# jeongminpark417/COALA-GNN

Measured on AMD Instinct MI355X. Metric: feature-gather GB/s (payload = rows x dim x 4 B delivered per second), IGB-medium GraphSAGE minibatch fetch, higher is better.
Workload: dtype f32

## Files before the change

coala-gnn_amd/csrc/coala_cache.hip:

```cpp
#include <hip/hip_runtime.h>
#include <hip/hip_ext.h>

#include <algorithm>
#include <cmath>
#include <cstdarg>
#include <cstdio>
#include <cstdlib>
#include <cstring>
#include <new>
#include <type_traits>
#include <utility>
#include <vector>

#include "../../include/coala_hip.h"
#include "coala_internal.h"

namespace {

constexpr uint64_t kEmptyKey = 0xFFFFFFFFFFFFFFFFull;
constexpr uint32_t kLinkMiss = 0x80000000u;
constexpr uint32_t kLinkBad = 0x7FFFFFFFu;
constexpr int kStatBlocks = 2048;
constexpr int kFillSlots = 8;

struct CacheDev {
    void* keys;
    uint64_t* set_cnt;
    uint32_t* color_meta;
    int32_t* color_counters;
    const int32_t* node_color;
    float* lines;
    const float* cold;
    uint64_t num_sets;
    uint64_t num_rows;
    uint32_t cache_dim;
    uint32_t dim;
    uint32_t n_gpus;
    int32_t gshift;
    int32_t sshift;
    uint32_t distributed;
    uint32_t cold_partitioned;
    uint32_t tag32;
    uint64_t* set_head;
    uint32_t* miss_link;
    unsigned long long* stats;
    uint32_t* miss_list;
    uint32_t list_sub;
};

constexpr int kListShards = 64;
constexpr int kListStride = 64;
constexpr int kStatWriteBad = 2 * kStatBlocks + kFillSlots + 1;
constexpr int kStatProbeBad = kStatWriteBad + 1;
constexpr int kStatHostWords = kStatProbeBad + 1;
constexpr int kStatList = (kStatHostWords + 31) & ~31;
constexpr int kStatWords = kStatList + 2 * kListShards * kListStride / 2;
__device__ __forceinline__ uint32_t* list_counter(const CacheDev& c, uint32_t parity, uint32_t shard) {
    return reinterpret_cast<uint32_t*>(c.stats + kStatList) + (parity * kListShards + shard) * kListStride;
}

__device__ __forceinline__ uint64_t set_of(const CacheDev& c, uint64_t id) {
    uint64_t k = id;
    if (c.distributed) {
        if (c.gshift >= 0) k = id >> c.gshift;
        else if ((id >> 32) == 0) k = (uint32_t)id / c.n_gpus;
        else k = id / c.n_gpus;
    }
    if (c.sshift >= 0) return k & (c.num_sets - 1);
    if ((k >> 32) == 0 && (c.num_sets >> 32) == 0) return (uint32_t)k % (uint32_t)c.num_sets;
    return k % c.num_sets;
}

__device__ __forceinline__ uint64_t cold_row_of(const CacheDev& c, uint64_t id) {
    if (!c.cold_partitioned) return id;
    if (c.gshift >= 0) return id >> c.gshift;
    return id / c.n_gpus;
}

constexpr int kMaxRanges = 64;
struct RangeSet {
    uint32_t n;
    uint32_t total;
    uint32_t begin[kMaxRanges];
    uint32_t vstart[kMaxRanges + 1];
};
__device__ __forceinline__ uint32_t pos_of(const RangeSet& rs, uint32_t v) {
    if (rs.n == 1) return v < rs.total ? rs.begin[0] + v : 0xFFFFFFFFu;
    uint32_t pos = 0xFFFFFFFFu;
    for (uint32_t k = 0; k < rs.n; ++k) {
        const uint32_t a = rs.vstart[k], b = rs.vstart[k + 1];
        if (v >= a && v < b) pos = rs.begin[k] + (v - a);
    }
    return pos;
}
struct Redirect {
    int64_t begin, end;
    float* out;
    const int64_t* row_map;
};

template <int CTRL> __device__ __forceinline__ uint32_t dpp_u32(uint32_t v) {
    return (uint32_t)__builtin_amdgcn_mov_dpp((int)v, CTRL, 0xF, 0xF, true);
}
__device__ __forceinline__ uint32_t umin_u32(uint32_t a, uint32_t b) { return a < b ? a : b; }
__device__ __forceinline__ uint64_t readlane64(uint64_t v, int src_lane) {
    uint32_t lo = __builtin_amdgcn_readlane((int)(uint32_t)v, src_lane);
    uint32_t hi = __builtin_amdgcn_readlane((int)(uint32_t)(v >> 32), src_lane);
    return ((uint64_t)hi << 32) | lo;
}

__device__ __forceinline__ uint64_t shfl64(uint64_t v, int src) {
    const uint32_t lo = __shfl((int)(uint32_t)v, src), hi = __shfl((int)(uint32_t)(v >> 32), src);
    return ((uint64_t)hi << 32) | lo;
}

typedef float vfloat4 __attribute__((ext_vector_type(4)));
typedef unsigned long long vu64x2 __attribute__((ext_vector_type(2)));
typedef unsigned int vu32x4 __attribute__((ext_vector_type(4)));

template <typename TAG> struct TagGeo;
template <> struct TagGeo<uint64_t> {
    using vec = vu64x2;
    static constexpr int KPL = 2;
    static constexpr int LPS = 16;
    static constexpr int SPL = 4;
    static constexpr uint64_t EMPTY = 0xFFFFFFFFFFFFFFFFull;
};
template <> struct TagGeo<uint32_t> {
    using vec = vu32x4;
    static constexpr int KPL = 4;
    static constexpr int LPS = 8;
    static constexpr int SPL = 8;
    static constexpr uint32_t EMPTY = 0xFFFFFFFFu;
};
template <int VEC> struct VecT;
template <> struct VecT<4> { using type = vfloat4; };
template <> struct VecT<1> { using type = float; };

template <int CD, int VEC, int NP = 4>
struct Geo {
    static constexpr int UNITS = CD / VEC;
    static constexpr int LPR = UNITS >= 64 ? 64 : UNITS;
    static constexpr int RPP = 64 / LPR;
    static constexpr int VPL = UNITS / LPR;
    static constexpr int PASSES = (VPL >= 16) ? 1 : NP;
    static constexpr int R = RPP * PASSES;
};

constexpr int kK1MinWaves = 4;
constexpr int kK1Passes = 4;
constexpr int64_t kK1SingleMaxChunks = 1 << 20;
constexpr int kK1Waves = 2;
#ifdef COALA_DEV_KNOBS
constexpr int kK1MaxWaves = 4;
#else
constexpr int kK1MaxWaves = kK1Waves;
#endif

template <typename V> __device__ __forceinline__ V nt_load(const V* p) { return __builtin_nontemporal_load(p); }
template <typename V> __device__ __forceinline__ void nt_store(V v, V* p) { __builtin_nontemporal_store(v, p); }

template <int CD, int VEC, typename TAG, int NP, bool FULL, bool REDIR, bool SINGLE>
__global__ __launch_bounds__(64 * kK1MaxWaves, kK1MinWaves) void probe_gather_kernel(const int64_t* __restrict__ idx, float* __restrict__ out,
                                                                    int64_t n, uint32_t gen, uint32_t n_blocks, CacheDev c, Redirect rd) {
    using G = Geo<CD, VEC, NP>;
    using V = typename VecT<VEC>::type;
    using TG = TagGeo<TAG>;
    using TV = typename TG::vec;
    constexpr int R = G::R;
    static_assert(R <= 32, "per-chunk row masks are 32 bits wide");
    if (blockIdx.x == 0 && threadIdx.x < kFillSlots) reinterpret_cast<uint32_t*>(c.stats + 2 * kStatBlocks)[(gen & 1u) * kFillSlots + threadIdx.x] = 0u;
    uint32_t* fill_flag = reinterpret_cast<uint32_t*>(c.stats + 2 * kStatBlocks) + 2 * kFillSlots;
    if (blockIdx.x == 0 && threadIdx.x == kFillSlots) fill_flag[(gen + 1u) & 1u] = 0u;
    if (blockIdx.x == 0 && threadIdx.x < kListShards) *list_counter(c, (gen + 1u) & 1u, threadIdx.x) = 0u;
    constexpr int TSTEPS = (R + TG::SPL - 1) / TG::SPL;
    int lane = threadIdx.x & 63;
#ifdef COALA_DEV_KNOBS
    const int wpb = (int)(blockDim.x >> 6);
#else
    constexpr int wpb = kK1Waves;
#endif
    const int64_t wave = (int64_t)blockIdx.x * wpb + (threadIdx.x >> 6);
    const int64_t n_waves = (int64_t)n_blocks * wpb;
    const int64_t n_chunks = (n + R - 1) / R;
    const uint32_t nunits = c.dim / VEC;
    const TAG* __restrict__ keys = reinterpret_cast<const TAG*>(c.keys);

    struct Ids { uint64_t id[TSTEPS]; bool valid[TSTEPS]; int32_t drow[REDIR ? TSTEPS : 1]; };
    struct Tags { uint64_t id[TSTEPS]; uint32_t set[TSTEPS]; TV kk[TSTEPS]; bool ok[TSTEPS]; bool valid[TSTEPS]; int32_t drow[REDIR ? TSTEPS : 1]; };
    auto load_ids = [&](int64_t chunk) {
        Ids r;
#pragma unroll
        for (int t = 0; t < TSTEPS; ++t) {
            const int q_l = t * TG::SPL + lane / TG::LPS;
            const int64_t i_l = chunk * R + q_l;
            r.valid[t] = (chunk < n_chunks) && (q_l < R) && (i_l < n);
            r.id[t] = r.valid[t] ? (uint64_t)idx[i_l] : 0;
            if (REDIR) {
                int32_t d = -1;
                if (r.valid[t] && i_l >= rd.begin && i_l < rd.end) d = (int32_t)(rd.row_map ? rd.row_map[i_l - rd.begin] : i_l - rd.begin);
                r.drow[t] = d;
            }
        }
        return r;
    };
    auto load_tags = [&](const Ids& ids) {
        Tags r;
#pragma unroll
        for (int t = 0; t < TSTEPS; ++t) {
            r.id[t] = ids.id[t];
            r.valid[t] = ids.valid[t];
            if (REDIR) r.drow[t] = ids.drow[t];
            r.ok[t] = ids.valid[t] && ids.id[t] < c.num_rows;
            r.set[t] = r.ok[t] ? (uint32_t)set_of(c, ids.id[t]) : 0u;
            r.kk[t] = TV(TG::EMPTY);
            if (r.ok[t]) r.kk[t] = *reinterpret_cast<const TV*>(keys + (uint64_t)r.set[t] * COALA_WAYS + (lane % TG::LPS) * TG::KPL);
        }
        return r;
    };

    int64_t chunk = wave;
    Ids ids_next = load_ids(chunk);
    Tags tags = load_tags(ids_next);
    if (!SINGLE) ids_next = load_ids(chunk + n_waves);

    for (; chunk < n_chunks; chunk += n_waves) {
        asm volatile("" : "+v"(lane));
        const int64_t base = chunk * R;
        uint32_t slot_v[TSTEPS];
        int32_t drow_v[REDIR ? TSTEPS : 1];
        uint64_t hit_b[TSTEPS], bad_b[TSTEPS];
        bool lead_l[TSTEPS], imiss_l[TSTEPS], bad_l[TSTEPS];
        unsigned long long prev[TSTEPS];
        const uint32_t lane_way0 = (uint32_t)((lane % TG::LPS) * TG::KPL);
#pragma unroll
        for (int t = 0; t < TSTEPS; ++t) {
            const TAG want = (TAG)tags.id[t];
            uint32_t way = 0xFFu;
#pragma unroll
            for (int k = TG::KPL - 1; k >= 0; --k)
                if (tags.kk[t][k] == want) way = lane_way0 + (uint32_t)k;
            if (!tags.ok[t]) way = 0xFFu;
            way = umin_u32(way, dpp_u32<0xB1>(way));
            way = umin_u32(way, dpp_u32<0x4E>(way));
            way = umin_u32(way, dpp_u32<0x141>(way));
            if (TG::LPS == 16) way = umin_u32(way, dpp_u32<0x140>(way));
            const bool hit = way != 0xFFu;
            slot_v[t] = tags.set[t] * COALA_WAYS + (way & (COALA_WAYS - 1));
            if (REDIR) drow_v[t] = tags.drow[t];
            hit_b[t] = __ballot(hit);
            bad_l[t] = tags.valid[t] && !tags.ok[t];
            bad_b[t] = __ballot(bad_l[t]);
            lead_l[t] = tags.valid[t] && (lane % TG::LPS) == 0;
            imiss_l[t] = lead_l[t] && tags.ok[t] && !hit;
            prev[t] = 0;
            if (imiss_l[t]) {
                const unsigned long long tag = ((unsigned long long)gen << 32) | (unsigned long long)(base + t * TG::SPL + lane / TG::LPS + 1);
                prev[t] = atomicExch(reinterpret_cast<unsigned long long*>(c.set_head + tags.set[t]), tag);
            }
        }
        {
            bool any = false;
#pragma unroll
            for (int t = 0; t < TSTEPS; ++t) any = any || imiss_l[t] || bad_l[t];
            if (__ballot(any) != 0 && lane == 0) fill_flag[gen & 1u] = 1u;
        }
        const uint32_t shard = (uint32_t)chunk & (kListShards - 1);
        uint32_t list_at = 0;
        if (c.list_sub) {
            uint32_t n_miss = 0, n_bad = 0;
#pragma unroll
            for (int t = 0; t < TSTEPS; ++t) {
                n_miss += (uint32_t)__builtin_popcountll(__ballot(imiss_l[t]));
                n_bad += (uint32_t)__builtin_popcountll(__ballot(bad_l[t] && lead_l[t]));
            }
            if (n_miss && lane == 0) list_at = atomicAdd(list_counter(c, gen & 1u, shard), n_miss);
            if (n_bad && lane == 0) atomicAdd(c.stats + kStatProbeBad, (unsigned long long)n_bad);
        }
        auto row_slot = [&](int q) { return (uint32_t)__builtin_amdgcn_readlane((int)slot_v[q / TG::SPL], TG::LPS * (q % TG::SPL)); };
        auto row_hit = [&](int q) { return ((hit_b[q / TG::SPL] >> (TG::LPS * (q % TG::SPL))) & 1) != 0; };
        auto row_bad = [&](int q) { return ((bad_b[q / TG::SPL] >> (TG::LPS * (q % TG::SPL))) & 1) != 0; };
        Ids ids_next2;
        if (!SINGLE) ids_next2 = load_ids(chunk + 2 * n_waves);

        const int sub = (G::RPP == 2) ? (lane >> 5) : 0;
        const int l_in = lane & (G::LPR - 1);
        V val[G::PASSES][G::VPL];
#pragma unroll
        for (int p = 0; p < G::PASSES; ++p) {
            const uint32_t s_a = row_slot(p * G::RPP), s_b = row_slot(p * G::RPP + (G::RPP - 1));
            const bool h_a = row_hit(p * G::RPP), h_b = row_hit(p * G::RPP + (G::RPP - 1));
            const uint32_t s = (G::RPP == 2 && sub) ? s_b : s_a;
            const bool h = (G::RPP == 2 && sub) ? h_b : h_a;
            const V* src = reinterpret_cast<const V*>(c.lines + (uint64_t)s * CD);
#pragma unroll
            for (int v = 0; v < G::VPL; ++v) {
                const uint32_t u = v * G::LPR + l_in;
                if (h && (FULL || u < nunits)) val[p][v] = nt_load(src + u);
            }
        }
        if (!SINGLE) {
            tags = load_tags(ids_next);
            ids_next = ids_next2;
        }
#pragma unroll
        for (int p = 0; p < G::PASSES; ++p) {
            const int q = p * G::RPP + sub;
            const bool h_a = row_hit(p * G::RPP), h_b = row_hit(p * G::RPP + (G::RPP - 1));
            const bool bad_a = row_bad(p * G::RPP), bad_b2 = row_bad(p * G::RPP + (G::RPP - 1));
            const bool h = (G::RPP == 2 && sub) ? h_b : h_a;
            const bool bad = (G::RPP == 2 && sub) ? bad_b2 : bad_a;
            V* dst = reinterpret_cast<V*>(out + (base + q) * (int64_t)c.dim);
            if (REDIR) {
                auto row_drow = [&](int r) { return (int32_t)__builtin_amdgcn_readlane(drow_v[r / TG::SPL], TG::LPS * (r % TG::SPL)); };
                const int32_t dr_a = row_drow(p * G::RPP), dr_b = row_drow(p * G::RPP + (G::RPP - 1));
                const int32_t dr = (G::RPP == 2 && sub) ? dr_b : dr_a;
                if (dr >= 0) dst = reinterpret_cast<V*>(rd.out + (int64_t)dr * (int64_t)c.dim);
            }
#pragma unroll
            for (int v = 0; v < G::VPL; ++v) {
                const uint32_t u = v * G::LPR + l_in;
                if (FULL || u < nunits) {
                    if (h) dst[u] = val[p][v];
                    else if (bad) dst[u] = V(0.0f);
                }
            }
        }
#pragma unroll
        for (int t = 0; t < TSTEPS; ++t) {
            if (lead_l[t]) {
                uint32_t w = 0u;
                if (imiss_l[t]) w = kLinkMiss | (((uint32_t)(prev[t] >> 32) == gen) ? (uint32_t)prev[t] : 0u);
                else if (bad_l[t]) w = kLinkBad;
                c.miss_link[base + t * TG::SPL + lane / TG::LPS] = w;
            }
        }
        if (c.list_sub) {
            uint32_t at = (uint32_t)__builtin_amdgcn_readfirstlane((int)list_at);
#pragma unroll
            for (int t = 0; t < TSTEPS; ++t) {
                const uint64_t mb = __ballot(imiss_l[t]);
                if (imiss_l[t]) c.miss_list[shard * c.list_sub + at + (uint32_t)__builtin_popcountll(mb & ((1ull << lane) - 1ull))] = (uint32_t)(base + t * TG::SPL + lane / TG::LPS);
                at += (uint32_t)__builtin_popcountll(mb);
            }
        }
        if (SINGLE) break;
    }
}

enum { kOpAssign = 0, kOpAdd = 1, kOpAdagrad = 2, kOpAdam = 3, kOpRowAdagrad = 4 };

struct WriteExtra {
    float* state2;
    int32_t* row_step;
    double ln_b1, ln_b2;
    double step;
    float b1, b2;
    float omb1, omb1_lo;
    float omb2;
};
struct AdamRow { float step_size, rsbc2; };

__device__ __forceinline__ float adam_op(float g, float old, float& m, float& v, const WriteExtra& ex, const AdamRow& r, float eps) {
    const float p = ex.omb1 * g;
    float e = __builtin_fmaf(ex.omb1, g, -p);
    e = __builtin_fmaf(ex.omb1_lo, g, e);
    const float mn = __builtin_fmaf(ex.b1, m, p) + e;
    const float vn = __builtin_fmaf(ex.b2, v, ex.omb2 * (g * g));
    m = mn;
    v = vn;
    return old - (r.step_size * mn) / __builtin_fmaf(__builtin_sqrtf(vn), r.rsbc2, eps);
}
__device__ __forceinline__ vfloat4 adam_op(vfloat4 g, vfloat4 old, vfloat4& m, vfloat4& v, const WriteExtra& ex, const AdamRow& r, float eps) {
    vfloat4 o;
#pragma unroll
    for (int k = 0; k < 4; ++k) {
        float mk = m[k], vk = v[k];
        o[k] = adam_op(g[k], old[k], mk, vk, ex, r, eps);
        m[k] = mk;
        v[k] = vk;
    }
    return o;
}
__device__ __forceinline__ float sq_acc(float x, float acc) { return __builtin_fmaf(x, x, acc); }
__device__ __forceinline__ float sq_acc(vfloat4 x, float acc) {
#pragma unroll
    for (int k = 0; k < 4; ++k) acc = __builtin_fmaf(x[k], x[k], acc);
    return acc;
}
__device__ __forceinline__ float scaled_sub(float x, float old, float scale) { return __builtin_fmaf(-scale, x, old); }
__device__ __forceinline__ vfloat4 scaled_sub(vfloat4 x, vfloat4 old, float scale) {
    vfloat4 o;
#pragma unroll
    for (int k = 0; k < 4; ++k) o[k] = __builtin_fmaf(-scale, x[k], old[k]);
    return o;
}

template <int OP> __device__ __forceinline__ float write_op(float x, float old, float& st, float a, float eps) {
    if (OP == kOpAssign) return x;
    if (OP == kOpAdd) return __builtin_fmaf(a, x, old);
    const float s = st + x * x;
    st = s;
    return old - a * x / (__builtin_sqrtf(s) + eps);
}
template <int OP> __device__ __forceinline__ vfloat4 write_op(vfloat4 x, vfloat4 old, vfloat4& st, float a, float eps) {
    vfloat4 r;
#pragma unroll
    for (int k = 0; k < 4; ++k) {
        float s = st[k];
        r[k] = write_op<OP>(x[k], old[k], s, a, eps);
        st[k] = s;
    }
    return r;
}

template <int CD, int VEC, typename TAG, int OP>
__global__ __launch_bounds__(256) void write_rows_kernel(const int64_t* __restrict__ ids, const float* __restrict__ src, float* __restrict__ state,
                                                         int64_t n, float a, float eps, CacheDev c, WriteExtra ex) {
    using G = Geo<CD, VEC, 1>;
    using V = typename VecT<VEC>::type;
    using TG = TagGeo<TAG>;
    using TV = typename TG::vec;
    constexpr int R = TG::SPL;
    static_assert(R % G::RPP == 0, "a chunk is a whole number of passes");
    const int lane = threadIdx.x & 63;
// ... 59 lines not shown
            if (OP == kOpAdam) {
                double t = ex.step;
                if (ex.row_step) {
                    const int32_t t0 = ex.row_step[id];
                    const int32_t t1 = t0 < 0x7FFFFFFF ? t0 + 1 : t0;
                    if (l_in == 0) ex.row_step[id] = t1;
                    t = (double)t1;
                }
                const double bc1 = -expm1(t * ex.ln_b1), bc2 = -expm1(t * ex.ln_b2);
                ar.step_size = (float)((double)a / bc1);
                ar.rsbc2 = (float)(1.0 / sqrt(bc2));
            }
            float scale = 0.0f;
            if (OP == kOpRowAdagrad) {
                float part = 0.0f;
#pragma unroll
                for (int v = 0; v < G::VPL; ++v) part = sq_acc(x[v], part);
#pragma unroll
                for (int d = 1; d < G::LPR; d <<= 1) part += __shfl_xor(part, d);
                float s = 0.0f;
                if (act) s = state[id] + part / (float)c.dim;
                if (act && l_in == 0) state[id] = s;
                scale = a / (__builtin_sqrtf(s) + eps);
            }
#pragma unroll
            for (int v = 0; v < G::VPL; ++v) {
                const uint32_t u = v * G::LPR + l_in;
                if (u < nunits && act) {
                    V nv;
                    if (OP == kOpAdam) {
                        nv = adam_op(x[v], old[v], st[v], st2[v], ex, ar, eps);
                        st_row[u] = st[v];
                        st2_row[u] = st2[v];
                    } else if (OP == kOpRowAdagrad) {
                        nv = scaled_sub(x[v], old[v], scale);
                    } else {
                        nv = write_op<OP>(x[v], old[v], st[v], a, eps);
                        if (OP == kOpAdagrad) st_row[u] = st[v];
                    }
                    cold_row[u] = nv;
                    for (uint32_t mm = m; mm; mm &= mm - 1)
                        reinterpret_cast<V*>(set_lines + (uint64_t)__builtin_ctz(mm) * CD)[u] = nv;
                }
            }
        }
    }
}



__device__ __forceinline__ void rank_row(const CacheDev& c, uint32_t gen, uint32_t pos, uint64_t id, uint32_t& slot, uint32_t& win) {
    const uint64_t set = set_of(c, id);
    uint32_t cur = (uint32_t)c.set_head[set];
    uint32_t total = 0, rank = 0;
    while (cur) {
        const uint32_t p2 = cur - 1;
        ++total;
        rank += (p2 < pos) ? 1u : 0u;
        cur = c.miss_link[p2] & ~kLinkMiss;
    }
    const uint64_t cv = __hip_atomic_load(c.set_cnt + set, __ATOMIC_RELAXED, __HIP_MEMORY_SCOPE_AGENT);
    const uint32_t cnt0 = ((uint32_t)(cv >> 32) == gen) ? (uint32_t)cv - total : (uint32_t)cv;
    if (rank == 0) __hip_atomic_store(c.set_cnt + set, ((uint64_t)gen << 32) | (uint32_t)(cnt0 + total), __ATOMIC_RELAXED, __HIP_MEMORY_SCOPE_AGENT);
    const uint32_t way = (cnt0 + rank) & (COALA_WAYS - 1);
    slot = (uint32_t)(set * COALA_WAYS) + way;
    win = (rank + COALA_WAYS >= total) ? 1u : 0u;
    if (win) {
        if (c.tag32) reinterpret_cast<uint32_t*>(c.keys)[slot] = (uint32_t)id;
        else reinterpret_cast<uint64_t*>(c.keys)[slot] = id;
        if (c.color_counters) {
            const int32_t col = c.node_color[id];
            atomicSub(c.color_counters + c.color_meta[slot], 1);
            atomicAdd(c.color_counters + col, 1);
            c.color_meta[slot] = (uint32_t)col;
        }
    }
}
template <typename G, typename V>
__device__ __forceinline__ void cold_load(const CacheDev& c, const uint64_t (&id)[G::PASSES], const bool (&live)[G::PASSES], int l_in, uint32_t nunits,
                                          V (&val)[G::PASSES][G::VPL]) {
#pragma unroll
    for (int p = 0; p < G::PASSES; ++p) {
        const V* src = reinterpret_cast<const V*>(c.cold + cold_row_of(c, id[p]) * (uint64_t)c.dim);
#pragma unroll
        for (int v = 0; v < G::VPL; ++v) {
            const uint32_t u = v * G::LPR + l_in;
            if (live[p] && u < nunits) val[p][v] = nt_load(src + u);
        }
    }
}
template <int CD, typename G, typename V>
__device__ __forceinline__ void fill_store(const CacheDev& c, V* const (&dst)[G::PASSES], const uint32_t (&slot)[G::PASSES], const bool (&winner)[G::PASSES],
                                           const bool (&live)[G::PASSES], int l_in, uint32_t nunits, const V (&val)[G::PASSES][G::VPL]) {
#pragma unroll
    for (int p = 0; p < G::PASSES; ++p) {
        V* line = reinterpret_cast<V*>(c.lines + (uint64_t)slot[p] * CD);
#pragma unroll
        for (int v = 0; v < G::VPL; ++v) {
            const uint32_t u = v * G::LPR + l_in;
            if (live[p] && u < nunits) {
                nt_store(val[p][v], dst[p] + u);
                if (winner[p]) nt_store(val[p][v], line + u);
            }
        }
    }
}
__device__ __forceinline__ void add_block_stats(const CacheDev& c, uint32_t my_miss, uint32_t my_bad) {
    __shared__ uint32_t s_m[256 / 64], s_b[256 / 64];
    const int lane = threadIdx.x & 63;
    for (int off = 32; off > 0; off >>= 1) { my_miss += __shfl_down(my_miss, off); my_bad += __shfl_down(my_bad, off); }
    if (lane == 0) { s_m[threadIdx.x >> 6] = my_miss; s_b[threadIdx.x >> 6] = my_bad; }
    __syncthreads();
    if (threadIdx.x == 0) {
        uint32_t m = 0, b = 0;
        for (int w = 0; w < (int)(blockDim.x >> 6); ++w) { m += s_m[w]; b += s_b[w]; }
        if (m) c.stats[2 * blockIdx.x] += m;
        if (b) c.stats[2 * blockIdx.x + 1] += b;
    }
}

template <int CD, int VEC, bool REDIR = false, int NP = 4>
__global__ __launch_bounds__(256) void miss_fill_kernel(CacheDev c, const int64_t* __restrict__ idx, float* __restrict__ out,
                                                        int tile_rows, int sparse_max, uint32_t gen, RangeSet rs, Redirect rd, int dyn_slot) {
    using G = Geo<CD, VEC, NP>;
    using V = typename VecT<VEC>::type;
    constexpr int R = G::R;
    const int lane = threadIdx.x & 63;
    const int64_t wave = (int64_t)blockIdx.x * (blockDim.x >> 6) + (threadIdx.x >> 6);
    const int64_t n_waves = (int64_t)gridDim.x * (blockDim.x >> 6);
    const int64_t n_tiles = ((int64_t)rs.total + tile_rows - 1) / tile_rows;
    const int chunks_per_tile = tile_rows / R;
    const uint32_t nunits = c.dim / VEC;
    const int sub = (G::RPP == 2) ? (lane >> 5) : 0;
    const int l_in = lane & (G::LPR - 1);
    uint32_t my_miss = 0, my_bad = 0;

    constexpr int U = 8;
    uint32_t* ticket = reinterpret_cast<uint32_t*>(c.stats + 2 * kStatBlocks) + (dyn_slot < 0 ? 0 : dyn_slot);
    const bool dyn = dyn_slot >= 0;
    if (reinterpret_cast<const uint32_t*>(c.stats + 2 * kStatBlocks)[2 * kFillSlots + (gen & 1u)] == 0u) return;
    const int64_t n_deal = dyn ? 1 : n_waves;
    const int64_t even8 = n_tiles / (n_waves * 8);
    const int claim_min = even8 < 1 ? 1 : (even8 > U ? U : (int)even8);
    int claim = claim_min;
    for (int64_t unit = dyn ? -1 : wave;;) {
      int64_t claim_end = n_tiles;
      if (dyn) {
          uint32_t t = 0;
          if (lane == 0) t = atomicAdd(ticket, (uint32_t)claim);
          unit = (int64_t)(uint32_t)__builtin_amdgcn_readfirstlane((int)t);
          if (unit >= n_tiles) break;
          claim_end = unit + claim < n_tiles ? unit + claim : n_tiles;
          claim = claim * 2 > 4 * U ? 4 * U : claim * 2;
      } else if (unit >= n_tiles) break;
     for (int64_t tile0 = unit; tile0 < claim_end; tile0 += n_deal * U) {
      const int n_here = dyn ? (int)(claim_end - tile0 < U ? claim_end - tile0 : U) : U;
      uint64_t st_pack = 0;
#pragma unroll
      for (int u = 0; u < U; ++u) {
          const int64_t tile = tile0 + u * n_deal;
          const uint32_t p = (u < n_here && tile < n_tiles && lane < tile_rows) ? pos_of(rs, (uint32_t)(tile * tile_rows + lane)) : 0xFFFFFFFFu;
          const uint32_t w = (p != 0xFFFFFFFFu) ? c.miss_link[p] : 0u;
          const uint64_t v = (w == 0u) ? 0u : ((w & kLinkMiss) ? 1u : 2u);
          st_pack |= v << (8 * u);
      }
      if (!__ballot(st_pack != 0)) continue;
// ... 64 lines not shown
          uint64_t m_sel = 0;
#pragma unroll
          for (int u = 0; u < U; ++u) {
              const uint32_t cnt = (uint32_t)__builtin_popcountll(mmask[u]);
              if (u_sel < 0) {
                  if (k < cnt) { u_sel = u; m_sel = mmask[u]; }
                  else k -= cnt;
              }
          }
          if (u_sel >= 0) {
              for (uint32_t i = 0; i < k; ++i) m_sel &= m_sel - 1;
              const uint32_t pos = pos_of(rs, (uint32_t)((tile0 + u_sel * n_deal) * tile_rows + __builtin_ctzll(m_sel)));
              rank_at(pos);
          }
          stream_holders(total_miss >= 64 ? ~0ull : ((1ull << total_miss) - 1ull));
          continue;
      }
#pragma nounroll
      for (int u = 0; u < U; ++u) {
        const uint8_t st = (uint8_t)(st_pack >> (8 * u));
        const uint64_t tile_mask = __ballot(st == 1);
        if (!tile_mask) continue;
        const uint32_t pos_l = st ? pos_of(rs, (uint32_t)((tile0 + u * n_deal) * tile_rows + lane)) : 0u;
        if (__builtin_popcountll(tile_mask) <= sparse_max) {
            if (st == 1) rank_at(pos_l);
            stream_holders(tile_mask);
        } else {
            int srcl[G::PASSES];
            bool live[G::PASSES];
            for (int ck = 0; ck < chunks_per_tile; ++ck) {
                const uint32_t live_mask = (uint32_t)(tile_mask >> (ck * R)) & ((1u << R) - 1u);
                if (!live_mask) continue;
                const int lane0 = ck * R;
                if (st == 1 && lane >= lane0 && lane < lane0 + R) rank_at(pos_l);
#pragma unroll
                for (int p = 0; p < G::PASSES; ++p) {
                    const int q = p * G::RPP + sub;
                    live[p] = (live_mask >> q) & 1;
                    srcl[p] = lane0 + q;
                }
                move_group(srcl, live);
            }
        }
      }
     }
      if (!dyn) break;
    }
    add_block_stats(c, my_miss, my_bad);
}

template <int CD, int VEC, int NP = 4>
__global__ __launch_bounds__(256) void miss_fill_list_kernel(CacheDev c, const int64_t* __restrict__ idx, float* __restrict__ out, uint32_t gen) {
    using G = Geo<CD, VEC, NP>;
    using V = typename VecT<VEC>::type;
    constexpr int R = G::R;
    const int lane = threadIdx.x & 63;
    const uint32_t wave = blockIdx.x * (blockDim.x >> 6) + (threadIdx.x >> 6);
    const uint32_t n_waves = gridDim.x * (blockDim.x >> 6);
    const uint32_t nunits = c.dim / VEC;
    const int sub = (G::RPP == 2) ? (lane >> 5) : 0;
    const int l_in = lane & (G::LPR - 1);
    static_assert(kListShards == 64, "one list counter per lane");
    const uint32_t cnt_l = __hip_atomic_load(list_counter(c, gen & 1u, (uint32_t)lane), __ATOMIC_RELAXED, __HIP_MEMORY_SCOPE_AGENT);
    uint32_t incl = cnt_l;
    for (int off = 1; off < 64; off <<= 1) {
        const uint32_t v = __shfl_up(incl, off);
        if (lane >= off) incl += v;
    }
    const uint32_t excl = incl - cnt_l;
    const uint32_t total = (uint32_t)__builtin_amdgcn_readlane((int)incl, 63);
    if (total == 0) return;
    const uint32_t n_groups = (total + R - 1) / R;
    uint32_t* ticket = reinterpret_cast<uint32_t*>(c.stats + 2 * kStatBlocks) + (gen & 1u) * kFillSlots;
    uint32_t my_miss = 0;
    for (uint32_t g = wave; g < n_groups;) {
        uint32_t pos_l = 0;
#pragma unroll
        for (int j = 0; j < R; ++j) {
            const uint32_t e = g * R + j;
            const uint32_t s = (uint32_t)__builtin_popcountll(__ballot(incl <= e)) & 63u;
            const uint32_t off = e - (uint32_t)__builtin_amdgcn_readlane((int)excl, (int)s);
            if (lane == j && e < total) pos_l = c.miss_list[s * c.list_sub + off];
        }
        const bool have = lane < R && g * R + (uint32_t)lane < total;
        const uint64_t id_l = have ? (uint64_t)idx[pos_l] : 0;
        uint64_t id[G::PASSES];
        uint32_t pos[G::PASSES];
        bool live[G::PASSES];
        V val[G::PASSES][G::VPL];
#pragma unroll
        for (int p = 0; p < G::PASSES; ++p) {
            const int q = p * G::RPP + sub;
            live[p] = g * R + (uint32_t)q < total;
            id[p] = shfl64(id_l, q);
            pos[p] = (uint32_t)__shfl((int)pos_l, q);
        }
        cold_load<G>(c, id, live, l_in, nunits, val);
        uint32_t t = 0;
        if (lane == 0) t = atomicAdd(ticket, 1u);
        uint32_t slot_l = 0, win_l = 0;
        if (have) rank_row(c, gen, pos_l, id_l, slot_l, win_l);
        uint32_t slot[G::PASSES];
        bool winner[G::PASSES];
        V* dst[G::PASSES];
#pragma unroll
        for (int p = 0; p < G::PASSES; ++p) {
            const int q = p * G::RPP + sub;
            slot[p] = (uint32_t)__shfl((int)slot_l, q);
            winner[p] = __shfl((int)win_l, q) != 0;
            dst[p] = reinterpret_cast<V*>(out + (uint64_t)pos[p] * c.dim);
        }
        fill_store<CD, G>(c, dst, slot, winner, live, l_in, nunits, val);
        if (lane == 0) my_miss += (total - g * R < (uint32_t)R) ? total - g * R : (uint32_t)R;
        g = n_waves + (uint32_t)__builtin_amdgcn_readfirstlane((int)t);
    }
    add_block_stats(c, my_miss, 0u);
}

template <int CD, int VEC, int NP = 4>
__global__ __launch_bounds__(256) void scatter_rows_kernel(float* __restrict__ out, const float* __restrict__ src,
                                                           const int64_t* __restrict__ map, RangeSet rs, uint32_t dim) {
    using G = Geo<CD, VEC, NP>;
    using V = typename VecT<VEC>::type;
    constexpr int R = G::R;
    const int lane = threadIdx.x & 63;
    const int64_t wave = (int64_t)blockIdx.x * (blockDim.x >> 6) + (threadIdx.x >> 6);
    const int64_t n_waves = (int64_t)gridDim.x * (blockDim.x >> 6);
    const int64_t n_chunks = ((int64_t)rs.total + R - 1) / R;
    const uint32_t nunits = dim / VEC;
    const int sub = (G::RPP == 2) ? (lane >> 5) : 0;
    const int l_in = lane & (G::LPR - 1);
    for (int64_t chunk = wave; chunk < n_chunks; chunk += n_waves) {
        const int64_t base = chunk * R;
        V val[G::PASSES][G::VPL];
        int64_t d[G::PASSES];
#pragma unroll
        for (int p = 0; p < G::PASSES; ++p) {
            const int64_t vr = base + p * G::RPP + sub;
            const uint32_t r = (vr < (int64_t)rs.total) ? pos_of(rs, (uint32_t)vr) : 0xFFFFFFFFu;
            d[p] = (r != 0xFFFFFFFFu) ? map[r] : -1;
            const V* s = reinterpret_cast<const V*>(src + (int64_t)r * (int64_t)dim);
#pragma unroll
            for (int v = 0; v < G::VPL; ++v) {
                const uint32_t u = v * G::LPR + l_in;
                if (d[p] >= 0 && u < nunits) val[p][v] = nt_load(s + u);
            }
        }
#pragma unroll
        for (int p = 0; p < G::PASSES; ++p) {
            V* t = reinterpret_cast<V*>(out + d[p] * (int64_t)dim);
#pragma unroll
            for (int v = 0; v < G::VPL; ++v) {
                const uint32_t u = v * G::LPR + l_in;
                if (d[p] >= 0 && u < nunits) nt_store(val[p][v], t + u);
            }
        }
    }
}

constexpr int kRouteItems = 4;
constexpr int kRouteTile = 64 * kRouteItems;

__device__ __forceinline__ uint32_t owner_of(uint64_t id, uint32_t n_parts, int pshift) {
    if (pshift >= 0) return (uint32_t)id & (n_parts - 1);
    if ((id >> 32) == 0) return (uint32_t)id % n_parts;
    return (uint32_t)(id % n_parts);
}

__global__ __launch_bounds__(256) void route_count_kernel(const int64_t* __restrict__ idx, int64_t n, uint32_t n_parts,
                                                          int pshift, uint32_t* __restrict__ wave_counts, int64_t n_tiles) {
    const int lane = threadIdx.x & 63;
    const int64_t tile = (int64_t)blockIdx.x * (blockDim.x >> 6) + (threadIdx.x >> 6);
    if (tile >= n_tiles) return;
    uint32_t mine = 0;
    for (int j = 0; j < kRouteItems; ++j) {
        const int64_t i = tile * kRouteTile + j * 64 + lane;
        const bool valid = i < n;
        const uint32_t o = valid ? owner_of((uint64_t)idx[i], n_parts, pshift) : 0xFFFFFFFFu;
        for (uint32_t g = 0; g < n_parts; ++g) {
            const uint64_t mask = __ballot(o == g);
            if ((uint32_t)lane == g) mine += (uint32_t)__builtin_popcountll(mask);
        }
    }
    if ((uint32_t)lane < n_parts) wave_counts[tile * n_parts + lane] = mine;
}

__global__ __launch_bounds__(1024) void route_scan_kernel(uint32_t* __restrict__ wave_counts, int64_t n_tiles, uint32_t n_parts,
                                                          int64_t bucket_stride, int64_t* __restrict__ counts_out,
                                                          int64_t* __restrict__ offsets_out, int64_t* __restrict__ bases) {
    __shared__ int64_t totals[64];
    const int lane = threadIdx.x & 63;
    const uint32_t n_waves = blockDim.x >> 6;
    for (uint32_t g = threadIdx.x >> 6; g < n_parts; g += n_waves) {
        uint32_t carry = 0;
        for (int64_t t0 = 0; t0 < n_tiles; t0 += 64) {
            const int64_t t = t0 + lane;
            const uint32_t c = (t < n_tiles) ? wave_counts[t * n_parts + g] : 0u;
            uint32_t incl = c;
            for (int off = 1; off < 64; off <<= 1) {
                const uint32_t v = __shfl_up(incl, off);
                if (lane >= off) incl += v;
            }
            if (t < n_tiles) wave_counts[t * n_parts + g] = carry + incl - c;
            carry += __shfl(incl, 63);
        }
        if (lane == 0) totals[g] = (int64_t)carry;
    }
    __syncthreads();
    if (threadIdx.x == 0) {
        int64_t acc = 0;
        for (uint32_t g = 0; g < n_parts; ++g) {
            counts_out[g] = totals[g];
            const int64_t b = bucket_stride > 0 ? (int64_t)g * bucket_stride : acc;
            bases[g] = b;
            if (offsets_out) offsets_out[g] = b;
            acc += totals[g];
        }
        if (offsets_out) offsets_out[n_parts] = bucket_stride > 0 ? (int64_t)n_parts * bucket_stride : acc;
    }
}

__global__ __launch_bounds__(256) void route_scatter_kernel(const int64_t* __restrict__ idx, int64_t n, uint32_t n_parts,
                                                            int pshift, const uint32_t* __restrict__ wave_offsets,
                                                            const int64_t* __restrict__ bases, int64_t* __restrict__ node_out,
                                                            int64_t* __restrict__ map_out, int64_t n_tiles) {
    const int lane = threadIdx.x & 63;
    const int64_t tile = (int64_t)blockIdx.x * (blockDim.x >> 6) + (threadIdx.x >> 6);
    if (tile >= n_tiles) return;
    int64_t off = 0;
    if ((uint32_t)lane < n_parts) off = bases[lane] + (int64_t)wave_offsets[tile * n_parts + lane];
    for (int j = 0; j < kRouteItems; ++j) {
        const int64_t i = tile * kRouteTile + j * 64 + lane;
        const bool valid = i < n;
        const int64_t id = valid ? idx[i] : 0;
        const uint32_t o = valid ? owner_of((uint64_t)id, n_parts, pshift) : 0xFFFFFFFFu;
        int64_t dest = -1;
        for (uint32_t g = 0; g < n_parts; ++g) {
            const uint64_t mask = __ballot(o == g);
            const int64_t bg = __shfl(off, (int)g);
            if (o == g) dest = bg + __builtin_popcountll(mask & ((1ull << lane) - 1ull));
            if ((uint32_t)lane == g) off += __builtin_popcountll(mask);
        }
        if (valid) {
            node_out[dest] = id;
            map_out[dest] = i;
        }
    }
}

}


namespace {

struct LaunchShape {
    int k1_grid_cap;
    int k1_waves;
    bool k1_single;
    int k1_passes;
    int k2_grid_cap;
    int k2_tile_rows;
    int k2_sparse_max;
    int k2_unit_tiles;
};

LaunchShape launch_shape(uint32_t cache_dim, bool host_tier) {
    LaunchShape s;
    s.k1_grid_cap = 16384;
    s.k1_waves = kK1Waves;
    s.k1_single = cache_dim >= 256;
    s.k1_passes = 0;
    const int host_blocks = std::min(64, std::max(24, 16 * 1024 / (int)cache_dim));
    s.k2_grid_cap = host_tier ? host_blocks : kStatBlocks;
    s.k2_tile_rows = host_tier ? 64 : 0;
    s.k2_sparse_max = host_tier ? 32 : 0;
    s.k2_unit_tiles = host_tier ? 1 : 0;
    return s;
}

#ifdef COALA_DEV_KNOBS
void apply_dev_knobs(LaunchShape& s) {
    if (const char* e = getenv("COALA_K1_PASSES")) { int v = atoi(e); if (v == 2 || v == 4 || v == 8 || v == 16) s.k1_passes = v; }
    if (const char* e = getenv("COALA_K1_GRID")) { int g = atoi(e); if (g >= 1 && g <= 65535) s.k1_grid_cap = g; }
    if (const char* e = getenv("COALA_K1_WAVES")) { int w = atoi(e); if (w == 1 || w == 2 || w == 4) s.k1_waves = w; }
    if (const char* e = getenv("COALA_K1_SINGLE")) s.k1_single = atoi(e) != 0;
    if (const char* e = getenv("COALA_K2_TILE_ROWS")) { int t = atoi(e); if (t == 0 || t == 8 || t == 16 || t == 32 || t == 64) s.k2_tile_rows = t; }
    if (const char* e = getenv("COALA_K2_GRID")) { int g = atoi(e); if (g >= 1 && g <= kStatBlocks) s.k2_grid_cap = g; }
    if (const char* e = getenv("COALA_K2_SPARSE")) { int g = atoi(e); if (g >= 0 && g <= 64) s.k2_sparse_max = g; }
    if (const char* e = getenv("COALA_K2_UNIT_TILES")) { int g = atoi(e); if (g >= 0 && g <= 1) s.k2_unit_tiles = g; }
}
#endif

}

struct coala_cache {
    coala_cache_config_t cfg;
    CacheDev d;
    uint64_t cap = 0;
    uint32_t gen = 0;
    int32_t* node_color_dev = nullptr;
    uint32_t* wave_counts = nullptr;
    uint64_t wave_counts_cap = 0;
    int64_t* route_bases = nullptr;
    struct EvPair { hipEvent_t a, b; int kind; uint64_t rows; };
    std::vector<EvPair> ev_live;
    std::vector<hipEvent_t> ev_pool;
    coala_cache_profile_t prof{};
    hipStream_t last_stream = nullptr;
    hipStream_t order_stream = nullptr;
    bool order_set = false;
    hipEvent_t order_ev = nullptr;
    uint64_t table_bytes = 0;
    LaunchShape shape;
    bool host_tier = false;
    int32_t* color_pin = nullptr;
    int32_t* color_pin_async = nullptr;
    hipEvent_t color_ev = nullptr;
    int32_t color_pending = -1;
    int64_t open_batch_rows = -1;
    std::vector<std::pair<int64_t, int64_t>> open_filled;
    int64_t open_filled_rows = 0;
    Redirect open_redirect{0, 0, nullptr, nullptr};
    int fill_launches = 0;
    uint64_t rows_total = 0;
    uint64_t cum_hit = 0, cum_miss = 0;
    uint64_t prof_hit0 = 0, prof_miss0 = 0;
    bool fetch_events = false;
    static constexpr int kFetchRing = 2048;
    std::vector<hipEvent_t> fev;
    uint64_t fev_calls = 0;
    hipEvent_t last_begin = nullptr, last_end = nullptr;
};

namespace {

#define fail coala_fail_
#define HIPCHK COALA_HIPCHK

int follow_stream(coala_cache* h, hipStream_t s) {
    if (h->order_set && h->order_stream != s) {
        if (!h->order_ev) HIPCHK(hipEventCreateWithFlags(&h->order_ev, hipEventDisableTiming));
        if (hipEventRecord(h->order_ev, h->order_stream) == hipSuccess) HIPCHK(hipStreamWaitEvent(s, h->order_ev, 0));
        else (void)hipGetLastError();
    }
    h->order_stream = s;
    h->order_set = true;
    return COALA_OK;
}

int ilog2_exact(uint64_t v) {
    if (v == 0 || (v & (v - 1))) return -1;
    int s = 0;
    while ((1ull << s) != v) ++s;
    return s;
}

int ensure_scratch(coala_cache* h, uint64_t n, hipStream_t s) {
    if (n <= h->cap) return COALA_OK;
    HIPCHK(hipStreamSynchronize(s));
    uint64_t cap = h->cap ? h->cap : 1024;
    while (cap < n) cap *= 2;
    if (h->d.miss_link) HIPCHK(hipFree(h->d.miss_link));
    h->d.miss_link = nullptr;
    HIPCHK(hipMalloc((void**)&h->d.miss_link, cap * sizeof(uint32_t)));
    if (h->d.miss_list) HIPCHK(hipFree(h->d.miss_list));
    h->d.miss_list = nullptr;
    h->d.list_sub = (uint32_t)(cap / kListShards) + 32u;
    HIPCHK(hipMalloc((void**)&h->d.miss_list, (uint64_t)kListShards * h->d.list_sub * sizeof(uint32_t)));
// ... 274 lines not shown
    out->reserved = 0;
    return COALA_OK;
}

enum { kPhaseProbe = 1, kPhaseFill = 2, kPhaseBoth = 3 };

static int read_feature_impl(coala_cache_t* h, float* out, const int64_t* idx, int64_t n, void* stream, bool force_dist,
                             int phases, const int64_t* begins, const int64_t* ends, int n_ranges,
                             const coala_row_redirect_t* redirect, hipEvent_t ext_begin = nullptr, hipEvent_t ext_end = nullptr,
                             hipEvent_t* rode = nullptr) {
    if (rode) rode[0] = rode[1] = nullptr;
    if (!h) return fail(COALA_EINVAL, "null handle");
    h->last_begin = h->last_end = nullptr;
    if (n < 0 || n > 0x7FFFFFFFll) return fail(COALA_EINVAL, "n=%lld out of range", (long long)n);
    if (phases & kPhaseProbe) {
        if (h->open_batch_rows >= 0)
            return fail(COALA_EINVAL, "a batch of %lld rows is still open (%lld filled): finish its serve_fill calls or call coala_cache_serve_abort",
                        (long long)h->open_batch_rows, (long long)h->open_filled_rows);
    } else if (h->open_batch_rows != n || h->gen == 0) {
        return fail(COALA_EINVAL, "serve_fill without a matching serve_probe (batch of %lld rows, probe saw %lld)", (long long)n, (long long)h->open_batch_rows);
    }
    if (n == 0) return COALA_OK;
    if (!idx || (!out && !(redirect && redirect->begin == 0 && redirect->end == n))) return fail(COALA_EINVAL, "null buffer");
    Redirect rd{0, 0, nullptr, nullptr};
    if (phases & kPhaseProbe) {
        if (redirect && redirect->end > redirect->begin) {
            if (redirect->begin < 0 || redirect->end > n || !redirect->out)
                return fail(COALA_EINVAL, "redirect [%lld, %lld) outside the batch of %lld rows, or null destination", (long long)redirect->begin, (long long)redirect->end, (long long)n);
            rd = Redirect{redirect->begin, redirect->end, redirect->out, redirect->row_map};
        }
    } else {
        rd = h->open_redirect;
    }
    const int64_t whole_b = 0, whole_e = n;
    if (phases == kPhaseBoth) { begins = &whole_b; ends = &whole_e; n_ranges = 1; }
    int64_t fill_rows = 0;
    if (phases & kPhaseFill) {
        if (n_ranges < 0 || (n_ranges > 0 && (!begins || !ends))) return fail(COALA_EINVAL, "bad fill ranges");
        std::vector<std::pair<int64_t, int64_t>> add;
        for (int k = 0; k < n_ranges; ++k) {
            if (begins[k] < 0 || begins[k] > ends[k] || ends[k] > n)
                return fail(COALA_EINVAL, "fill range [%lld, %lld) outside the batch of %lld rows", (long long)begins[k], (long long)ends[k], (long long)n);
            if (ends[k] > begins[k]) add.emplace_back(begins[k], ends[k]);
        }
        if (phases == kPhaseFill) {
            std::vector<std::pair<int64_t, int64_t>> all = h->open_filled;
            all.insert(all.end(), add.begin(), add.end());
            std::sort(all.begin(), all.end());
            for (size_t k = 1; k < all.size(); ++k)
                if (all[k].first < all[k - 1].second)
                    return fail(COALA_EINVAL, "fill range [%lld, %lld) overlaps positions that were already filled in this batch", (long long)all[k].first, (long long)all[k].second);
            h->open_filled.swap(all);
        }
        for (auto& r : add) fill_rows += r.second - r.first;
        if (fill_rows == 0 && !(phases & kPhaseProbe)) return COALA_OK;
    }
    hipStream_t s = (hipStream_t)stream;
    HIPCHK(hipSetDevice(h->cfg.device));
    if (int rc_ = follow_stream(h, s)) return rc_;
    int rc = ensure_scratch(h, (uint64_t)n, s);
    if (rc) return rc;
    if (phases & kPhaseProbe) {
        h->fill_launches = 0;
        if (++h->gen == 0) {
            HIPCHK(hipMemsetAsync(h->d.set_head, 0, h->d.num_sets * 8, s));
            HIPCHK(hipMemset2DAsync(reinterpret_cast<char*>(h->d.set_cnt) + 4, 8, 0, 4, h->d.num_sets, s));
            HIPCHK(hipMemsetAsync(h->d.stats + kStatList, 0, (size_t)(kStatWords - kStatList) * 8, s));
            h->gen = 1;
        }
        if (!(phases & kPhaseFill)) {
            h->open_batch_rows = n;
            h->open_filled.clear();
            h->open_filled_rows = 0;
            h->open_redirect = rd;
        }
    }
    const uint32_t gen = h->gen;
    const bool redir = rd.end > rd.begin;
    const bool vec4 = (h->d.dim % 4 == 0) && aligned16(out) && aligned16(h->d.cold) && (!redir || aligned16(rd.out));
    CacheDev d = h->d;
    if (force_dist) d.distributed = 1u;
    const bool list_form = phases == kPhaseBoth && h->host_tier;
    if (!list_form) d.list_sub = 0;
    hipEvent_t fe_begin = nullptr, fe_end = nullptr;
    if (h->fetch_events && phases == kPhaseBoth && !(h->cfg.flags & COALA_FLAG_PROFILE)) {
        if (h->fev.empty()) h->fev.assign(2 * (size_t)coala_cache::kFetchRing, nullptr);
        const size_t slot = (size_t)(h->fev_calls % coala_cache::kFetchRing);
        for (size_t k = 2 * slot; k < 2 * slot + 2; ++k)
            if (!h->fev[k]) HIPCHK(hipEventCreate(&h->fev[k]));
        fe_begin = h->fev[2 * slot];
        fe_end = h->fev[2 * slot + 1];
    }
    const bool own_ring = fe_begin != nullptr;
    if (!own_ring && !(h->cfg.flags & COALA_FLAG_PROFILE)) {
        fe_begin = (phases & kPhaseProbe) ? ext_begin : nullptr;
        fe_end = (phases & kPhaseFill) ? ext_end : nullptr;
    }
    int n_sets = 0, set_no = 0;
    if ((phases & kPhaseFill) && fill_rows > 0) {
        int live = 0;
        for (int k = 0; k < n_ranges; ++k) live += ends[k] > begins[k];
        n_sets = (live + kMaxRanges - 1) / kMaxRanges;
    }
    rc = dispatch_geo(d.cache_dim, vec4, [&](auto geo) -> int {
        constexpr int CD = geo_cd(geo);
        constexpr int VEC = geo_vec(geo);
        using G = Geo<CD, VEC>;
        if (phases & kPhaseProbe) {
            ProfScope ps(h, s, 0, (uint64_t)n, fe_begin, nullptr);
            if (rode) rode[0] = ps.on ? ps.a : fe_begin;
            const bool full = (VEC == 4) && ((int)d.dim == CD);
            auto launch_k1 = [&](auto tag_c, auto np_c) {
                using TAG = decltype(tag_c);
                constexpr int NP = decltype(np_c)::value;
                constexpr int NPR = (Geo<CD, VEC, NP>::R > 8) ? NP / 2 : NP;
                using GK = Geo<CD, VEC, NP>;
                using GR = Geo<CD, VEC, NPR>;
                const int64_t chunks = redir ? (n + GR::R - 1) / GR::R : (n + GK::R - 1) / GK::R;
                const LaunchShape& ls = h->shape;
                const bool single = ls.k1_single && chunks <= kK1SingleMaxChunks;
                const dim3 grid(grid_for(chunks, ls.k1_waves, single ? (int)((kK1SingleMaxChunks + ls.k1_waves - 1) / ls.k1_waves) : ls.k1_grid_cap)), block(64 * ls.k1_waves);
                auto pick = [&](auto single_c) {
                    constexpr bool S = decltype(single_c)::value;
                    if (redir) return full ? probe_gather_kernel<CD, VEC, TAG, NPR, true, true, S> : probe_gather_kernel<CD, VEC, TAG, NPR, false, true, S>;
                    return full ? probe_gather_kernel<CD, VEC, TAG, NP, true, false, S> : probe_gather_kernel<CD, VEC, TAG, NP, false, false, S>;
                };
                ps.launch(single ? pick(std::true_type{}) : pick(std::false_type{}), grid, block, idx, out, n, gen, (uint32_t)grid.x, d, rd);
            };
#ifdef COALA_DEV_KNOBS
            if (h->shape.k1_passes) {
                auto by_np = [&](auto tag_c) {
                    switch (h->shape.k1_passes) {
                        case 2: launch_k1(tag_c, std::integral_constant<int, 2>{}); break;
                        case 8: launch_k1(tag_c, std::integral_constant<int, 8>{}); break;
                        case 16: launch_k1(tag_c, std::integral_constant<int, (Geo<CD, VEC, 16>::R <= 32 ? 16 : 8)>{}); break;
                        default: launch_k1(tag_c, std::integral_constant<int, 4>{}); break;
                    }
                };
                if (d.tag32) by_np(uint32_t{}); else by_np(uint64_t{});
            } else
#endif
            if (d.tag32) launch_k1(uint32_t{}, std::integral_constant<int, kK1Passes>{});
            else launch_k1(uint64_t{}, std::integral_constant<int, kK1Passes>{});
        }
        if ((phases & kPhaseFill) && fill_rows > 0) {
            if (list_form) {
                ProfScope ps(h, s, 2, 0, nullptr, fe_end);
                if (rode) rode[1] = ps.on ? ps.b : fe_end;
                h->fill_launches++;
                ps.launch(miss_fill_list_kernel<CD, VEC>, dim3(grid_for((n + G::R - 1) / G::R, 4, h->shape.k2_grid_cap)), dim3(256), d, idx, out, gen);
                return COALA_OK;
            }
            const int tile_rows = h->shape.k2_tile_rows > 0 ? h->shape.k2_tile_rows : G::R;
            return for_each_range_set(begins, ends, n_ranges, [&](const RangeSet& rs) -> int {
                const bool last_set = ++set_no == n_sets;
                ProfScope ps(h, s, 2, 0, nullptr, last_set ? fe_end : nullptr);
                if (rode && last_set) rode[1] = ps.on ? ps.b : fe_end;
                const int64_t tiles = ((int64_t)rs.total + tile_rows - 1) / tile_rows;
                const dim3 grid(grid_for(tiles, 4, h->shape.k2_grid_cap));
                const int64_t waves = (int64_t)grid.x * 4;
                int dyn_slot = -1;
                if (h->shape.k2_unit_tiles > 0 && tiles > waves && tiles < 0x7FFFFFFF && h->fill_launches < kFillSlots)
                    dyn_slot = (int)((gen & 1u) * kFillSlots) + h->fill_launches;
                h->fill_launches++;
                if (redir) ps.launch(miss_fill_kernel<CD, VEC, true>, grid, dim3(256), d, idx, out, tile_rows, h->shape.k2_sparse_max, gen, rs, rd, dyn_slot);
                else ps.launch(miss_fill_kernel<CD, VEC, false>, grid, dim3(256), d, idx, out, tile_rows, h->shape.k2_sparse_max, gen, rs, rd, dyn_slot);
                return COALA_OK;
            });
        }
        return COALA_OK;
    });
    if (rc) return rc;
    if (own_ring) {
        h->last_begin = fe_begin;
        h->last_end = fe_end;
        h->fev_calls++;
    }
    if (phases & kPhaseProbe) h->rows_total += (uint64_t)n;
    if (phases == kPhaseFill) {
        h->open_filled_rows += fill_rows;
        if (h->open_filled_rows == h->open_batch_rows) {
            h->open_batch_rows = -1;
            h->open_filled.clear();
            h->open_filled_rows = 0;
        }
    }
    HIPCHK(hipGetLastError());
    if (h->cfg.flags & COALA_FLAG_SYNC) HIPCHK(hipStreamSynchronize(s));
    return COALA_OK;
}

int coala_cache_read_feature(coala_cache_t* h, float* out, const int64_t* idx, int64_t n, void* stream) {
    return read_feature_impl(h, out, idx, n, stream, false, kPhaseBoth, nullptr, nullptr, 0, nullptr);
}

int coala_cache_serve(coala_cache_t* h, float* out, const int64_t* ids, int64_t n, void* stream) {
    return read_feature_impl(h, out, ids, n, stream, true, kPhaseBoth, nullptr, nullptr, 0, nullptr);
}

int coala_cache_serve_probe(coala_cache_t* h, float* out, const int64_t* ids, int64_t n, void* stream) {
    return read_feature_impl(h, out, ids, n, stream, true, kPhaseProbe, nullptr, nullptr, 0, nullptr);
}

int coala_cache_serve_probe_redirect(coala_cache_t* h, float* out, const int64_t* ids, int64_t n, const coala_row_redirect_t* redirect,
                                     void* stream) {
    return read_feature_impl(h, out, ids, n, stream, true, kPhaseProbe, nullptr, nullptr, 0, redirect);
}

int coala_serve_probe_redirect_ev_(coala_cache_t* h, float* out, const int64_t* ids, int64_t n, const coala_row_redirect_t* redirect, void* stream,
                                   hipEvent_t begin_ev, hipEvent_t* rode) {
// ... 312 lines not shown
```

Measured before the change: 82.64.

## Gather early-chunk misses directly from cold tier in probe kernel

For the first few chunks (about 512 KB of payload), the probe/gather kernel now loads missed rows straight from the cold (host) tier into the output, instead of leaving them for the fill kernel. Miss-list entries from these chunks carry a flag so the fill kernel reads the row back from the output buffer rather than refetching it from the cold tier. The intent is to start slow host-tier traffic earlier and overlap it with the probe pass. The cost is extra per-row branching, 64-bit readlanes and divergent cold loads in the hot kernel.

```diff
diff --git a/coala-gnn_amd/csrc/coala_cache.hip b/coala-gnn_amd/csrc/coala_cache.hip
--- a/coala-gnn_amd/csrc/coala_cache.hip
+++ b/coala-gnn_amd/csrc/coala_cache.hip
@@ -46,7 +46,9 @@
     unsigned long long* stats;
     uint32_t* miss_list;
     uint32_t list_sub;
+    uint32_t early_chunks;
 };
+constexpr uint32_t kListEarly = 0x80000000u;
 
 constexpr int kListShards = 64;
 constexpr int kListStride = 64;
@@ -150,6 +152,8 @@
 constexpr int kK1MinWaves = 4;
 constexpr int kK1Passes = 4;
 constexpr int64_t kK1SingleMaxChunks = 1 << 20;
+constexpr int kK1EarlyBytes = 512 * 1024;
+constexpr int kK1EarlyMaxChunks = 128;
 constexpr int kK1Waves = 2;
 #ifdef COALA_DEV_KNOBS
 constexpr int kK1MaxWaves = 4;
@@ -227,9 +231,12 @@
     for (; chunk < n_chunks; chunk += n_waves) {
         asm volatile("" : "+v"(lane));
         const int64_t base = chunk * R;
+        const bool early = !REDIR && chunk < (int64_t)c.early_chunks;
         uint32_t slot_v[TSTEPS];
         int32_t drow_v[REDIR ? TSTEPS : 1];
+        uint64_t id_v[REDIR ? 1 : TSTEPS];
         uint64_t hit_b[TSTEPS], bad_b[TSTEPS];
+        uint64_t mov_b[TSTEPS];
         bool lead_l[TSTEPS], imiss_l[TSTEPS], bad_l[TSTEPS];
         unsigned long long prev[TSTEPS];
         const uint32_t lane_way0 = (uint32_t)((lane % TG::LPS) * TG::KPL);
@@ -249,6 +256,8 @@
             slot_v[t] = tags.set[t] * COALA_WAYS + (way & (COALA_WAYS - 1));
             if (REDIR) drow_v[t] = tags.drow[t];
             hit_b[t] = __ballot(hit);
+            if (!REDIR) id_v[t] = tags.id[t];
+            mov_b[t] = REDIR ? hit_b[t] : __ballot(hit || (early && tags.ok[t]));
             bad_l[t] = tags.valid[t] && !tags.ok[t];
             bad_b[t] = __ballot(bad_l[t]);
             lead_l[t] = tags.valid[t] && (lane % TG::LPS) == 0;
@@ -279,6 +288,8 @@
         }
         auto row_slot = [&](int q) { return (uint32_t)__builtin_amdgcn_readlane((int)slot_v[q / TG::SPL], TG::LPS * (q % TG::SPL)); };
         auto row_hit = [&](int q) { return ((hit_b[q / TG::SPL] >> (TG::LPS * (q % TG::SPL))) & 1) != 0; };
+        auto row_mov = [&](int q) { return ((mov_b[q / TG::SPL] >> (TG::LPS * (q % TG::SPL))) & 1) != 0; };
+        auto row_id = [&](int q) { return readlane64(id_v[REDIR ? 0 : q / TG::SPL], TG::LPS * (q % TG::SPL)); };
         auto row_bad = [&](int q) { return ((bad_b[q / TG::SPL] >> (TG::LPS * (q % TG::SPL))) & 1) != 0; };
         Ids ids_next2;
         if (!SINGLE) ids_next2 = load_ids(chunk + 2 * n_waves);
@@ -293,10 +304,18 @@
             const uint32_t s = (G::RPP == 2 && sub) ? s_b : s_a;
             const bool h = (G::RPP == 2 && sub) ? h_b : h_a;
             const V* src = reinterpret_cast<const V*>(c.lines + (uint64_t)s * CD);
+            bool m = h;
+            if (!REDIR) {
+                const uint64_t i_a = row_id(p * G::RPP), i_b = row_id(p * G::RPP + (G::RPP - 1));
+                const bool m_a = row_mov(p * G::RPP), m_b = row_mov(p * G::RPP + (G::RPP - 1));
+                const uint64_t i = (G::RPP == 2 && sub) ? i_b : i_a;
+                m = (G::RPP == 2 && sub) ? m_b : m_a;
+                if (!h) src = reinterpret_cast<const V*>(c.cold + cold_row_of(c, i) * (uint64_t)c.dim);
+            }
 #pragma unroll
             for (int v = 0; v < G::VPL; ++v) {
                 const uint32_t u = v * G::LPR + l_in;
-                if (h && (FULL || u < nunits)) val[p][v] = nt_load(src + u);
+                if (m && (FULL || u < nunits)) val[p][v] = nt_load(src + u);
             }
         }
         if (!SINGLE) {
@@ -306,7 +325,7 @@
 #pragma unroll
         for (int p = 0; p < G::PASSES; ++p) {
             const int q = p * G::RPP + sub;
-            const bool h_a = row_hit(p * G::RPP), h_b = row_hit(p * G::RPP + (G::RPP - 1));
+            const bool h_a = row_mov(p * G::RPP), h_b = row_mov(p * G::RPP + (G::RPP - 1));
             const bool bad_a = row_bad(p * G::RPP), bad_b2 = row_bad(p * G::RPP + (G::RPP - 1));
             const bool h = (G::RPP == 2 && sub) ? h_b : h_a;
             const bool bad = (G::RPP == 2 && sub) ? bad_b2 : bad_a;
@@ -340,7 +359,8 @@
 #pragma unroll
             for (int t = 0; t < TSTEPS; ++t) {
                 const uint64_t mb = __ballot(imiss_l[t]);
-                if (imiss_l[t]) c.miss_list[shard * c.list_sub + at + (uint32_t)__builtin_popcountll(mb & ((1ull << lane) - 1ull))] = (uint32_t)(base + t * TG::SPL + lane / TG::LPS);
+                if (imiss_l[t]) c.miss_list[shard * c.list_sub + at + (uint32_t)__builtin_popcountll(mb & ((1ull << lane) - 1ull))] =
+                    (uint32_t)(base + t * TG::SPL + lane / TG::LPS) | (early ? kListEarly : 0u);
                 at += (uint32_t)__builtin_popcountll(mb);
             }
         }
@@ -566,6 +586,20 @@
 #pragma unroll
     for (int p = 0; p < G::PASSES; ++p) {
         const V* src = reinterpret_cast<const V*>(c.cold + cold_row_of(c, id[p]) * (uint64_t)c.dim);
+#pragma unroll
+        for (int v = 0; v < G::VPL; ++v) {
+            const uint32_t u = v * G::LPR + l_in;
+            if (live[p] && u < nunits) val[p][v] = nt_load(src + u);
+        }
+    }
+}
+template <typename G, typename V>
+__device__ __forceinline__ void list_load(const CacheDev& c, const float* out, const uint64_t (&id)[G::PASSES], const uint32_t (&pos)[G::PASSES],
+                                          const bool (&early)[G::PASSES], const bool (&live)[G::PASSES], int l_in, uint32_t nunits, V (&val)[G::PASSES][G::VPL]) {
+#pragma unroll
+    for (int p = 0; p < G::PASSES; ++p) {
+        const float* row = early[p] ? out + (uint64_t)pos[p] * c.dim : c.cold + cold_row_of(c, id[p]) * (uint64_t)c.dim;
+        const V* src = reinterpret_cast<const V*>(row);
 #pragma unroll
         for (int v = 0; v < G::VPL; ++v) {
             const uint32_t u = v * G::LPR + l_in;
@@ -796,11 +830,13 @@
             const uint32_t off = e - (uint32_t)__builtin_amdgcn_readlane((int)excl, (int)s);
             if (lane == j && e < total) pos_l = c.miss_list[s * c.list_sub + off];
         }
+        const uint32_t early_l = pos_l & kListEarly;
+        pos_l &= ~kListEarly;
         const bool have = lane < R && g * R + (uint32_t)lane < total;
         const uint64_t id_l = have ? (uint64_t)idx[pos_l] : 0;
         uint64_t id[G::PASSES];
         uint32_t pos[G::PASSES];
-        bool live[G::PASSES];
+        bool live[G::PASSES], early[G::PASSES];
         V val[G::PASSES][G::VPL];
 #pragma unroll
         for (int p = 0; p < G::PASSES; ++p) {
@@ -808,8 +844,9 @@
             live[p] = g * R + (uint32_t)q < total;
             id[p] = shfl64(id_l, q);
             pos[p] = (uint32_t)__shfl((int)pos_l, q);
-        }
-        cold_load<G>(c, id, live, l_in, nunits, val);
+            early[p] = __shfl((int)early_l, q) != 0;
+        }
+        list_load<G>(c, out, id, pos, early, live, l_in, nunits, val);
         uint32_t t = 0;
         if (lane == 0) t = atomicAdd(ticket, 1u);
         uint32_t slot_l = 0, win_l = 0;
@@ -972,6 +1009,7 @@
     int k1_waves;
     bool k1_single;
     int k1_passes;
+    int k1_early_chunks;
     int k2_grid_cap;
     int k2_tile_rows;
     int k2_sparse_max;
@@ -984,6 +1022,8 @@
     s.k1_waves = kK1Waves;
     s.k1_single = cache_dim >= 256;
     s.k1_passes = 0;
+    const int chunk_bytes = (int)cache_dim * 4 * (cache_dim == 128 ? 8 : 4);
+    s.k1_early_chunks = host_tier ? std::min(kK1EarlyMaxChunks, kK1EarlyBytes / chunk_bytes) : 0;
     const int host_blocks = std::min(64, std::max(24, 16 * 1024 / (int)cache_dim));
     s.k2_grid_cap = host_tier ? host_blocks : kStatBlocks;
     s.k2_tile_rows = host_tier ? 64 : 0;
@@ -998,6 +1038,7 @@
     if (const char* e = getenv("COALA_K1_GRID")) { int g = atoi(e); if (g >= 1 && g <= 65535) s.k1_grid_cap = g; }
     if (const char* e = getenv("COALA_K1_WAVES")) { int w = atoi(e); if (w == 1 || w == 2 || w == 4) s.k1_waves = w; }
     if (const char* e = getenv("COALA_K1_SINGLE")) s.k1_single = atoi(e) != 0;
+    if (const char* e = getenv("COALA_K1_EARLY")) { long long v = atoll(e); if (v >= 0) s.k1_early_chunks = (int)std::min<long long>(v, 0x7FFFFFFF); }
     if (const char* e = getenv("COALA_K2_TILE_ROWS")) { int t = atoi(e); if (t == 0 || t == 8 || t == 16 || t == 32 || t == 64) s.k2_tile_rows = t; }
     if (const char* e = getenv("COALA_K2_GRID")) { int g = atoi(e); if (g >= 1 && g <= kStatBlocks) s.k2_grid_cap = g; }
     if (const char* e = getenv("COALA_K2_SPARSE")) { int g = atoi(e); if (g >= 0 && g <= 64) s.k2_sparse_max = g; }
@@ -1438,6 +1479,7 @@
     if (force_dist) d.distributed = 1u;
     const bool list_form = phases == kPhaseBoth && h->host_tier;
     if (!list_form) d.list_sub = 0;
+    d.early_chunks = list_form ? (uint32_t)h->shape.k1_early_chunks : 0u;
     hipEvent_t fe_begin = nullptr, fe_end = nullptr;
     if (h->fetch_events && phases == kPhaseBoth && !(h->cfg.flags & COALA_FLAG_PROFILE)) {
         if (h->fev.empty()) h->fev.assign(2 * (size_t)coala_cache::kFetchRing, nullptr);
@@ -1481,7 +1523,9 @@
                     if (redir) return full ? probe_gather_kernel<CD, VEC, TAG, NPR, true, true, S> : probe_gather_kernel<CD, VEC, TAG, NPR, false, true, S>;
                     return full ? probe_gather_kernel<CD, VEC, TAG, NP, true, false, S> : probe_gather_kernel<CD, VEC, TAG, NP, false, false, S>;
                 };
-                ps.launch(single ? pick(std::true_type{}) : pick(std::false_type{}), grid, block, idx, out, n, gen, (uint32_t)grid.x, d, rd);
+                CacheDev dk = d;
+                dk.early_chunks = (uint32_t)std::min<int64_t>((int64_t)d.early_chunks, chunks);
+                ps.launch(single ? pick(std::true_type{}) : pick(std::false_type{}), grid, block, idx, out, n, gen, (uint32_t)grid.x, dk, rd);
             };
 #ifdef COALA_DEV_KNOBS
             if (h->shape.k1_passes) {
```

Result: no change. 82.94 (median of 6 runs) (+0.4%).
